# forbes110/taiwan-whisper

Measured on AMD Instinct MI355X. Metric: distillation utterances/sec (30 s clips), higher is better.
Workload: dtype bf16

## Files before the change

### include/tw_hip.h

```cpp
#ifndef TW_HIP_H
#define TW_HIP_H
#include <stdint.h>
#ifdef __cplusplus
extern "C" {
#endif

typedef void* tw_stream_t;

#define TW_GEMM_BIAS 1
#define TW_GEMM_ROUND 2
#define TW_GEMM_GELU 4
#define TW_GEMM_RES 8
#define TW_GEMM_ACCUM 16
#define TW_GEMM_AUX_OUT 32
#define TW_GEMM_DGELU 64
#define TW_GEMM_TILE128 256
#define TW_GEMM_TILE256 512
#define TW_GEMM_TILE256x128 1024
#define TW_GEMM_TILE256PP 2048
#define TW_GEMM_NOSPLIT 16384
#define TW_GEMM_TILE256x128_S2 262144
#define TW_GEMM_GROUP_M(g) ((g) << 24)


int tw_gemm_bf16(const void* A, int64_t lda, int a_trans, const void* B, int64_t ldb, int b_trans, void* C,
                 int64_t ldc, int c_dtype, int M, int N, int K, int batch, int64_t sA, int64_t sB, int64_t sC,
                 float alpha, const void* bias, const void* res, int64_t ldr, int64_t sR, int res_dtype, int res_mod,
                 void* aux, int64_t ldaux, int64_t sAux, int flags, tw_stream_t stream);

int tw_gemm_route(const void* A, int64_t lda, int a_trans, const void* B, int64_t ldb, int b_trans, void* C,
                  int64_t ldc, int c_dtype, int M, int N, int K, int batch, int64_t sA, int64_t sB, int64_t sC,
                  const void* bias, const void* res, int64_t ldr, int64_t sR, int res_dtype, int res_mod, void* aux,
                  int64_t ldaux, int64_t sAux, int flags, int is_f16, int cus, int have_ws, int* out);

int tw_gemv_bf16(const void* x, int64_t ldx, const float* ln_w, const float* ln_b, float eps, const void* W,
                 int64_t ldw, void* C, int64_t ldc, int c_dtype, int M, int N, int K, const void* bias,
                 const void* res, int64_t ldr, int res_dtype, void* aux, int64_t ldaux, int flags,
                 void* kv_cache, int64_t kv_sb, int64_t kv_ld, int kv_col0, const int* t_dev, tw_stream_t stream);

int tw_layernorm_fwd(const void* x, int x_dtype, const float* w, const float* b, void* y, int y_dtype,
                     float* mean_out, float* rstd_out, int rows, int D, float eps, tw_stream_t stream);
int tw_add_layernorm_fwd(const void* x, int x_dtype, const void* r, void* x_out, const float* w, const float* b,
                         void* y, float* mean_out, float* rstd_out, int rows, int D, float eps, tw_stream_t stream);
int tw_layernorm_bwd(const void* x, int x_dtype, const float* w, const float* mean, const float* rstd, const void* dy,
                     int dy_dtype, float* dx, int dx_accum, float* dw_out, float* db_out, int rows, int D,
                     float* workspace, int64_t workspace_floats, tw_stream_t stream);
int tw_layernorm_bwd_ex(const void* x, int x_dtype, const float* w, const float* mean, const float* rstd, const void* dy,
                        int dy_dtype, float* dx, int dx_accum, float* dw_out, float* db_out, int rows, int D,
                        float* workspace, int64_t workspace_floats, void* g16, int g_dtype, tw_stream_t stream);

int tw_attn_fwd(const void* Q, int64_t ldq, const void* K, int64_t ldk, const void* V, int64_t ldv, void* O,
                int64_t ldo, float* lse, int B, int H, int Tq, int Tk, int head_dim, int causal, float scale,
                tw_stream_t stream);
int tw_attn_bwd(const void* Q, int64_t ldq, const void* K, int64_t ldk, const void* V, int64_t ldv, const void* O,
                int64_t ldo, const void* dO, int64_t lddo, const float* lse, void* dQ, int64_t lddq, void* dK,
                int64_t lddk, void* dV, int64_t lddv, int B, int H, int Tq, int Tk, int head_dim, int causal,
                float scale, float* workspace , tw_stream_t stream);
int tw_attn_fwd_varlen(const void* Q, int64_t ldq, const void* K, int64_t ldk, const void* V, int64_t ldv, void* O,
                       int64_t ldo, float* lse, const int* offq, const int* offk, int B, int H, int Mq, int max_q, int Tk,
                       int head_dim, int causal, float scale, tw_stream_t stream);
int tw_attn_fwd_varlen_f16(const void* Q, int64_t ldq, const void* K, int64_t ldk, const void* V, int64_t ldv, void* O,
                           int64_t ldo, float* lse, const int* offq, const int* offk, int B, int H, int Mq, int max_q,
                           int Tk, int head_dim, int causal, float scale, tw_stream_t stream);
int tw_attn_bwd_varlen(const void* Q, int64_t ldq, const void* K, int64_t ldk, const void* V, int64_t ldv,
                       const void* O, int64_t ldo, const void* dO, int64_t lddo, const float* lse, void* dQ,
                       int64_t lddq, void* dK, int64_t lddk, void* dV, int64_t lddv, const int* offq, const int* offk,
// ... 111 lines not shown
int tw_gelu_bwd_f32(const float* g, const float* pre, float* out, int64_t n, tw_stream_t stream);

#define TW_GEMM_CLAMP16 128
int tw_gemm_f16(const void* A, int64_t lda, int a_trans, const void* B, int64_t ldb, int b_trans, void* C,
                int64_t ldc, int c_dtype, int M, int N, int K, int batch, int64_t sA, int64_t sB, int64_t sC,
                float alpha, const void* bias, const void* res, int64_t ldr, int64_t sR, int res_dtype, int res_mod,
                void* aux, int64_t ldaux, int64_t sAux, int flags, tw_stream_t stream);
int tw_gemv_f16(const void* x, int64_t ldx, const float* ln_w, const float* ln_b, float eps, const void* W,
                int64_t ldw, void* C, int64_t ldc, int c_dtype, int M, int N, int K, const void* bias,
                const void* res, int64_t ldr, int res_dtype, void* aux, int64_t ldaux, int flags,
                void* kv_cache, int64_t kv_sb, int64_t kv_ld, int kv_col0, const int* t_dev, tw_stream_t stream);
int tw_attn_fwd_f16(const void* Q, int64_t ldq, const void* K, int64_t ldk, const void* V, int64_t ldv, void* O,
                    int64_t ldo, float* lse, int B, int H, int Tq, int Tk, int head_dim, int causal, float scale,
                    tw_stream_t stream);
int tw_mel_to_conv_input_f16(const float* mel, void* xt, int B, int nmel, int T, tw_stream_t stream);
int tw_attn_bwd_f16(const void* Q, int64_t ldq, const void* K, int64_t ldk, const void* V, int64_t ldv, const void* O,
                    int64_t ldo, const void* dO, int64_t lddo, const float* lse, void* dQ, int64_t lddq, void* dK,
                    int64_t lddk, void* dV, int64_t lddv, int B, int H, int Tq, int Tk, int head_dim, int causal,
                    float scale, float* workspace, tw_stream_t stream);
int tw_gelu_bwd_f16(const void* g, int g_dtype, const void* pre, void* out, int64_t n, tw_stream_t stream);
int tw_cast_f32_f16(const float* src, void* dst, int64_t n, tw_stream_t stream);
int tw_add_layernorm_fwd_f16(const void* x, int x_dtype, const void* r, void* x_out, const float* w, const float* b,
                             void* y, float* mean_out, float* rstd_out, int rows, int D, float eps, tw_stream_t stream);
int tw_adamw_ex(float* p, const float* g, float* m, float* v, void* p16, int p16_dtype, int64_t n, float lr, float b1,
                float b2, float eps, float wd, int step, const float* norm, float max_norm, float inv_scale,
                tw_stream_t stream);

int tw_flac_info(const uint8_t* data, int64_t n, int64_t* info);
int tw_flac_decode(const uint8_t* data, int64_t n, int32_t* out, int64_t cap, int64_t* frames);

#ifdef __cplusplus
}
#endif
#endif
```

### taiwan-whisper_amd/csrc/layernorm.hip

```cpp
#include "common.h"

#include <algorithm>

namespace {

constexpr int WPB = 4;

template <int VEC, int MAXJ, bool ADD = false, bool RH = false>
__global__ __launch_bounds__(256) void ln_fwd_kernel(const void* __restrict__ x, int x_dtype,
                                                     const float* __restrict__ w, const float* __restrict__ b,
                                                     void* __restrict__ y, int y_dtype, float* __restrict__ mean_out,
                                                     float* __restrict__ rstd_out, int rows, int D, float eps,
                                                     const bf16* __restrict__ r = nullptr, float* x_out = nullptr) {
  const int lane = lane_id();
  const int row = blockIdx.x * WPB + (threadIdx.x >> 6);
  if (row >= rows) return;
  const int J = D / (64 * VEC);
  const int64_t base = (int64_t)row * D;
  float v[MAXJ][VEC];
  float s = 0.f;
#pragma unroll
  for (int j = 0; j < MAXJ; ++j) {
    if (j < J) {
      const int e = (j * 64 + lane) * VEC;
      if constexpr (ADD) {
        const f32x4 t = *(const f32x4*)((const float*)x + base + e);
        const bf16x4 u = *(const bf16x4*)(r + base + e);
        const f32x4 o = f32x4{t[0] + e2f<RH>(u[0]), t[1] + e2f<RH>(u[1]), t[2] + e2f<RH>(u[2]), t[3] + e2f<RH>(u[3])};
        *(f32x4*)(x_out + base + e) = o;
        v[j][0] = o[0]; v[j][1] = o[1]; v[j][2] = o[2]; v[j][3] = o[3];
      } else if (VEC == 4) {
        if (x_dtype == TW_F32) {
          f32x4 t = *(const f32x4*)((const float*)x + base + e);
          v[j][0] = t[0]; v[j][1] = t[1]; v[j][2] = t[2]; v[j][3] = t[3];
        } else if (x_dtype == TW_BF16) {
          bf16x4 t = *(const bf16x4*)((const bf16*)x + base + e);
          v[j][0] = bf2f(t[0]); v[j][1] = bf2f(t[1]); v[j][2] = bf2f(t[2]); v[j][3] = bf2f(t[3]);
        } else {
          f16x4 t = *(const f16x4*)((const f16*)x + base + e);
          v[j][0] = (float)t[0]; v[j][1] = (float)t[1]; v[j][2] = (float)t[2]; v[j][3] = (float)t[3];
        }
      } else {
        v[j][0] = ld_as_f32(x, x_dtype, base + e);
      }
#pragma unroll
      for (int q = 0; q < VEC; ++q) s += v[j][q];
    }
  }
  const float mean = wave_sum(s) / D;
  float ss = 0.f;
#pragma unroll
  for (int j = 0; j < MAXJ; ++j)
// ... 315 lines not shown
      default: hipLaunchKernelGGL((ln_fwd_bf16_kernel<5, true>), g2, block, 0, stream, xb, w, b, yb, mean_out, rstd_out,
                                  rows, D, eps, rb, xo); break;
    }
  }
  TW_CHECK_LAUNCH();
  return TW_OK;
}

extern "C" int tw_add_layernorm_fwd_f16(const void* x, int x_dtype, const void* r, void* x_out, const float* w,
                                        const float* b, void* y, float* mean_out, float* rstd_out, int rows, int D,
                                        float eps, hipStream_t stream) {
  if (rows <= 0) return TW_OK;
  if (D % 256 || D > 1280) return TW_EUNSUPPORTED;
  if (x_dtype != TW_F32) return TW_EUNSUPPORTED;
  if ((((uintptr_t)x | (uintptr_t)r | (uintptr_t)x_out | (uintptr_t)y | (uintptr_t)w | (uintptr_t)b) & 15) != 0)
    return TW_EINVAL;
  hipLaunchKernelGGL((ln_fwd_kernel<4, 5, true, true>), dim3((rows + WPB - 1) / WPB), dim3(64 * WPB), 0, stream, x,
                     (int)TW_F32, w, b, y, (int)TW_F16, mean_out, rstd_out, rows, D, eps, (const bf16*)r,
                     (float*)x_out);
  TW_CHECK_LAUNCH();
  return TW_OK;
}

extern "C" int tw_layernorm_bwd_ex(const void* x, int x_dtype, const float* w, const float* mean, const float* rstd,
                                   const void* dy, int dy_dtype, float* dx, int dx_accum, float* dw_out,
                                   float* db_out, int rows, int D, float* workspace, int64_t workspace_floats,
                                   void* g16, int g_dtype, hipStream_t stream) {
  if (rows <= 0) return TW_OK;
  if (g16 && g_dtype != TW_BF16 && g_dtype != TW_F16) return TW_EINVAL;
  if (D % 64 || D > 1280) return TW_EUNSUPPORTED;
  int nblk = (rows + WPB - 1) / WPB;
  if (nblk > 1024) nblk = 1024;
  if (workspace_floats < (int64_t)nblk * 2 * D) return TW_EINVAL;
  const bool v4 = D % 256 == 0 && (((uintptr_t)x | (uintptr_t)dy | (uintptr_t)dx | (uintptr_t)w | (uintptr_t)g16) & 15) == 0;
#define TW_LN_BWD(J)                                                                                          \
  hipLaunchKernelGGL((ln_bwd_kernel<4, J>), dim3(nblk), dim3(256), 0, stream, x, x_dtype, w, mean, rstd, dy, dy_dtype, \
                     dx, dx_accum, workspace, rows, D, g16, g_dtype)
  if (v4 && D > 1024) {
    static const int cap = [] {
      int dev = 0, cus = 0, per = 0;
      (void)hipGetDevice(&dev);
      (void)hipDeviceGetAttribute(&cus, hipDeviceAttributeMultiprocessorCount, dev);
      (void)hipOccupancyMaxActiveBlocksPerMultiprocessor(&per, (const void*)ln_bwd_kernel<4, 5>, 256, 0);
      return std::max(1, cus) * std::max(1, per);
    }();
    if (nblk > cap) nblk = cap;
// ... 24 lines not shown
```

### taiwan-whisper_amd/tw/_native.py

```python
from __future__ import annotations

import ctypes
import os

_HERE = os.path.dirname(os.path.abspath(__file__))
LIB_PATH = os.environ.get("TW_HIP_LIB", os.path.join(_HERE, "_lib", "libtw_hip.so"))

P, I64, I32, F32 = ctypes.c_void_p, ctypes.c_int64, ctypes.c_int, ctypes.c_float

SIGNATURES = {
    "tw_gemm_bf16": [P, I64, I32, P, I64, I32, P, I64, I32, I32, I32, I32, I32, I64, I64, I64, F32, P,
                     P, I64, I64, I32, I32, P, I64, I64, I32, P],
    "tw_gemm_route": [P, I64, I32, P, I64, I32, P, I64, I32, I32, I32, I32, I32, I64, I64, I64, P,
                      P, I64, I64, I32, I32, P, I64, I64, I32, I32, I32, I32, P],
    "tw_flac_info": [P, I64, P],
    "tw_flac_decode": [P, I64, P, I64, P],
    "tw_gemv_bf16": [P, I64, P, P, F32, P, I64, P, I64, I32, I32, I32, I32, P, P, I64, I32, P, I64, I32,
                     P, I64, I64, I32, P, P],
    "tw_layernorm_fwd": [P, I32, P, P, P, I32, P, P, I32, I32, F32, P],
    "tw_layernorm_bwd": [P, I32, P, P, P, P, I32, P, I32, P, P, I32, I32, P, I64, P],
    "tw_layernorm_bwd_ex": [P, I32, P, P, P, P, I32, P, I32, P, P, I32, I32, P, I64, P, I32, P],
    "tw_add_layernorm_fwd": [P, I32, P, P, P, P, P, P, P, I32, I32, F32, P],
    "tw_attn_fwd": [P, I64, P, I64, P, I64, P, I64, P, I32, I32, I32, I32, I32, I32, F32, P],
    "tw_attn_bwd": [P, I64, P, I64, P, I64, P, I64, P, I64, P, P, I64, P, I64, P, I64, I32, I32, I32, I32,
                    I32, I32, F32, P, P],
    "tw_attn_fwd_varlen": [P, I64, P, I64, P, I64, P, I64, P, P, P, I32, I32, I32, I32, I32, I32, I32, F32, P],
    "tw_attn_fwd_varlen_f16": [P, I64, P, I64, P, I64, P, I64, P, P, P, I32, I32, I32, I32, I32, I32, I32, F32, P],
    "tw_attn_bwd_varlen": [P, I64, P, I64, P, I64, P, I64, P, I64, P, P, I64, P, I64, P, I64, P, P, I32, I32, I32,
                           I32, I32, I32, I32, F32, P, P],
    "tw_attn_bwd_varlen_f16": [P, I64, P, I64, P, I64, P, I64, P, I64, P, P, I64, P, I64, P, I64, P, P, I32, I32,
                               I32, I32, I32, I32, I32, F32, P, P],
    "tw_pack_plan": [P, I32, I32, P, P, P],
    "tw_embed_fwd_rows": [P, P, P, I32, P, I32, P, I32, I32, I32, I32, I32, P],
    "tw_pos_grad_rows": [P, P, I32, I32, I32, P, P],
    "tw_kl_ce": [P, P, I64, I32, P, I64, I32, F32, F32, F32, P, F32, P, P, P, P],
    "tw_logmel": [P, I32, P, P, P, P, P, P, P],
    "tw_logmel_len": [P, I32, I64, P, P, P, P, P, P, P],
    "tw_logmel_mels": [P, I32, I64, I32, P, P, P, P, P, P, P],
    "tw_mel_to_conv_input": [P, P, I32, I32, I32, P],
    "tw_embed_fwd": [P, P, I32, P, I32, P, I32, I32, I32, I32, I32, P],
    "tw_embed_bwd": [P, P, P, I32, I32, I64, P],
    "tw_cast_f32_bf16": [P, P, I64, P],
    "tw_transpose_bf16": [P, I64, I32, I32, P, I64, P],
    "tw_colsum": [P, I32, I64, I32, I32, P, I32, I32, P, I64, P],
    "tw_l2norm": [P, I64, P, P, P],
# ... 12 lines not shown
    "tw_spec_accept": [P, I32, P, I32, I64, P, P, P, P, P, P, P, P, P, I32, I32, P, P, P, I32, P],
    "tw_embed_step_multi": [P, P, I32, P, I32, P, I32, I32, I32, P, I32, P],
    "tw_embed_step_off": [P, P, I32, P, I32, P, I32, I32, I32, P, P, P],
    "tw_greedy_select": [P, I64, I32, I32, I32, P, P, I32, I64, P, P, I64, I32, P, P, I32, P],
    "tw_greedy_select_ts": [P, I64, I32, I32, I32, P, P, I64, P, P, I64, I32, P, P, I32, I32, I32, I32, P, P],
    "tw_select_sample": [P, I64, I32, I32, I32, P, P, I32, I64, P, P, I64, I32, P, P, I32, P, P, P],
    "tw_select_sample_ts": [P, I64, I32, I32, I32, P, P, I64, P, P, I64, I32, P, P, I32, I32, I32, I32, P, P, P, P],
    "tw_token_logprob": [P, I64, I32, I32, I32, I32, P, P],
    "tw_embed_step": [P, P, I32, P, I32, P, I32, I32, I32, P, P],
    "tw_kv_append": [P, I64, P, I64, I64, I32, I32, I32, P, P],
    "tw_kv_head_major": [P, I64, P, I32, I32, I32, I32, P],
    "tw_step_advance": [P, I32, P],
    "tw_gemm_f16": [P, I64, I32, P, I64, I32, P, I64, I32, I32, I32, I32, I32, I64, I64, I64, F32, P,
                    P, I64, I64, I32, I32, P, I64, I64, I32, P],
    "tw_gemv_f16": [P, I64, P, P, F32, P, I64, P, I64, I32, I32, I32, I32, P, P, I64, I32, P, I64, I32,
                    P, I64, I64, I32, P, P],
    "tw_attn_fwd_f16": [P, I64, P, I64, P, I64, P, I64, P, I32, I32, I32, I32, I32, I32, F32, P],
    "tw_mel_to_conv_input_f16": [P, P, I32, I32, I32, P],
    "tw_attn_bwd_f16": [P, I64, P, I64, P, I64, P, I64, P, I64, P, P, I64, P, I64, P, I64, I32, I32, I32, I32,
                        I32, I32, F32, P, P],
    "tw_gelu_bwd_f16": [P, I32, P, P, I64, P],
    "tw_cast_f32_f16": [P, P, I64, P],
    "tw_add_layernorm_fwd_f16": [P, I32, P, P, P, P, P, P, P, I32, I32, F32, P],
    "tw_adamw_ex": [P, P, P, P, P, I32, I64, F32, F32, F32, F32, F32, I32, P, F32, F32, P],
    "tw_gemm_f32": [P, I64, I32, P, I64, I32, P, I64, I32, I32, I32, I32, I64, I64, I64, I32, I64, I64, I64, F32,
                    P, P, I64, I64, I32, P, I64, I64, I32, P],
    "tw_attn_fwd_f32": [P, I64, P, I64, P, I64, P, I64, P, I32, I32, I32, I32, I32, I32, F32, P, I64, P],
    "tw_attn_bwd_f32": [P, I64, P, I64, P, I64, P, I64, P, I64, P, P, I64, P, I64, P, I64, I32, I32, I32, I32, I32,
                        I32, F32, P, I64, P],
    "tw_mel_to_conv_input_f32": [P, P, I32, I32, I32, P],
    "tw_im2col3_f32": [P, I64, P, I32, I32, I32, I32, P],
    "tw_gelu_bwd_f32": [P, P, P, I64, P],
}

STATUS = {1: "invalid argument / shape", 2: "unsupported configuration", 3: "HIP launch error"}

_lib = None


def lib():
    global _lib
    if _lib is None:
        if not os.path.exists(LIB_PATH):
            raise RuntimeError(f"tw: HIP library not built: {LIB_PATH} (run `make -C taiwan-whisper_amd` "
                               "or __graft_entry__.build()); there is no CPU fallback")
        l = ctypes.CDLL(LIB_PATH)
# ... 14 lines not shown
```

### taiwan-whisper_amd/tw/distill.py

```python
from __future__ import annotations

import contextlib
import math
import os
from typing import Optional

import torch

from . import ops as F
from .modeling import Backward, PackedRows, WhisperForConditionalGeneration, is_pseudo


def constant_with_warmup(step: int, warmup: int) -> float:
    if warmup > 0 and step < warmup:
        return step / warmup
    return 1.0


def linear_schedule(step: int, warmup: int, total: int) -> float:
    if warmup > 0 and step < warmup:
        return step / warmup
    return max(0.0, (total - step) / max(1, total - warmup))


# ... 43 lines not shown
            if self.growth_tracker == self.growth_interval:
                self.scale *= self.growth_factor
                self.growth_tracker = 0

    def state_dict(self):
        return {"scale": self.scale, "growth_factor": self.growth_factor, "backoff_factor": self.backoff_factor,
                "growth_interval": self.growth_interval, "_growth_tracker": self.growth_tracker}

    def load_state_dict(self, sd):
        self.scale = float(sd["scale"])
        self.growth_factor, self.backoff_factor = float(sd["growth_factor"]), float(sd["backoff_factor"])
        self.growth_interval = int(sd["growth_interval"])
        self.growth_tracker = int(sd["_growth_tracker"])


class DistillationTrainer:
    def __init__(self, student: WhisperForConditionalGeneration, teacher: WhisperForConditionalGeneration, *,
                 temperature: float = 2.0, kl_weight: float = 1.0, learning_rate: float = 1e-4,
                 adam_beta1: float = 0.9, adam_beta2: float = 0.999, adam_epsilon: float = 1e-8,
                 weight_decay: float = 0.0, max_grad_norm: float = 1.0, warmup_steps: int = 0,
                 lr_scheduler_type: str = "constant_with_warmup", max_steps: int = 0,
                 gradient_accumulation_steps: int = 1, freeze_encoder: bool = True, freeze_decoder: bool = False,
                 freeze_embed_positions: bool = True, process_group=None, dp_bucket_mb: int = 64,
                 overlap_update: Optional[bool] = None, force_exchange: bool = False):
        if student.compute != teacher.compute:
            raise ValueError(f"student computes in {student.compute}, teacher in {teacher.compute}: the reference "
                             "runs both under one mixed_precision setting")
        self.s, self.t = student, teacher
        self.temperature, self.kl_weight = temperature, kl_weight
        self.lr, self.b1, self.b2, self.eps = learning_rate, adam_beta1, adam_beta2, adam_epsilon
        self.wd, self.max_grad_norm = weight_decay, max_grad_norm
        self.warmup, self.sched, self.max_steps = warmup_steps, lr_scheduler_type, max_steps
        self.accum = gradient_accumulation_steps
        self.pg = process_group
        self.world = torch.distributed.get_world_size(process_group) if process_group is not None else 1
        self.force_exchange = bool(force_exchange) and process_group is not None
        self.dp = self.world > 1 or self.force_exchange
        self.bucket = dp_bucket_mb * (1 << 20) // 4
        self.fold_world = self.world & (self.world - 1) == 0
        self.overlap_update = (self.dp and freeze_encoder) if overlap_update is None else bool(overlap_update)
        if self.overlap_update and not freeze_encoder:
            raise ValueError("overlap_update needs a frozen encoder: the next forward must read no trainable weight")
        self.scaler = GradScaler() if student.compute == "fp16" else None
        if self.scaler is not None:
            if student.dtype != torch.float32:
                raise ValueError("fp16 distillation trains an fp32-master student under fp16 autocast")
            if overlap_update:
                raise ValueError("overlap_update: the fp16 loss scaler decides each update on the host")
            self.overlap_update = False
        self.pack_rows = student.compute != "fp32" and os.environ.get("TW_PACK_ROWS", "1") != "0"
        self._pin = {}
# ... 24 lines not shown
        return weight_decay_runs(self.s, self.wd, self.freeze_encoder, self.freeze_decoder)

    def num_trainable_parameters(self):
        return self.s.num_parameters(only_trainable=True)

    def lr_at(self, step):
        if self.sched == "linear":
            return self.lr * linear_schedule(step, self.warmup, self.max_steps)
        if self.sched == "constant":
            return self.lr
        return self.lr * constant_with_warmup(step, self.warmup)

    def _conv_input(self, batch):
        ci = batch.get("conv_input")
        if ci is not None and ci.dtype == self.s.act_dtype:
            return ci
        return self.s.conv_input(batch["input_features"])

    def _teacher_logits(self, conv_in, ids, labels, enc16, Tk, pk=None):
        t = self.t
        if self.share:
            t_ids = torch.empty_like(labels)
            F.shift_tokens_right(labels, t_ids, t.config.pad_token_id, t.config.decoder_start_token_id)
            ht = t.decode(t_ids if pk is None else pk.pack(t_ids), enc16, Tk, pk=pk)
        else:
            enc_t = t.encode(conv_in)
            ht = t.decode(ids if pk is None else pk.pack(ids), enc_t, Tk, pk=pk)
        return t.lm_head(ht)

    def _plan_rows(self, batch_labels, labels):
        B, T = labels.shape
        off = torch.empty(B + 1, dtype=torch.int32, device=labels.device)
        src = torch.empty(B * T, dtype=torch.int64, device=labels.device)
        F.pack_plan(labels, off, src)
        def descriptor(lens):
            pk = PackedRows(lens, off, src, T)
            return pk if pk.M > 0 else None

        if not batch_labels.is_cuda:
            pos = torch.arange(1, T + 1, dtype=torch.int64)
            lens = ((batch_labels >= 0) * pos).amax(1).tolist()
            return lambda: descriptor(lens)
        host = self._pin.get(B)
        if host is None:
            host = self._pin[B] = torch.empty(B + 1, dtype=torch.int32).pin_memory()
        host.copy_(off, non_blocking=True)
        ev = torch.cuda.Event()
        ev.record()

        def done():
            ev.synchronize()
            o = host.tolist()
            return descriptor([o[b + 1] - o[b] for b in range(B)])
        return done

    def train_step(self, batch, temperature: Optional[float] = None, end_of_dataloader: bool = False):
        T = self.temperature if temperature is None else temperature
        s = self.s
        conv_in = self._conv_input(batch)
        ids = batch["decoder_input_ids"].to(s.device).contiguous()
        labels = batch["labels"].to(s.device).contiguous()
        B, Td = ids.shape
        plan = self._plan_rows(batch["labels"], labels) if self.pack_rows else None
        enc_tape = [] if self.train_encoder else None
        enc16 = s.encode(conv_in, tape=enc_tape)
        self.flush()
        pk = plan() if plan is not None else None
        if self.micro == 0:
            s.grad.zero_()
        self._pending, self._reduced = [], []
        sync = self.micro + 1 == self.accum or end_of_dataloader
        self.bw.on_ready = self._grad_ready if (self.dp and sync) else None
        Tk = enc16.shape[0] // B
        tape = []
        with self._row_capacity(pk, B * Td):
            hs = s.decode(ids if pk is None else pk.pack(ids), enc16, Tk, tape=tape, pk=pk)
            ls = s.lm_head(hs)
            with torch.no_grad():
                lt = self._teacher_logits(conv_in, ids, labels, enc16, Tk, pk)
            lab = labels.reshape(-1) if pk is None else pk.pack(labels)
            F.count_valid(lab, self.nvalid)
            dlogits = ls
            gs = (self.scaler.scale if self.scaler is not None else 1.0) / (self.accum * (self.world if self.fold_world
                                                                                             else 1))
            out3, _ = F.kl_ce(ls, lt, lab, s.config.vocab_size, self.nvalid, T=T, ce_w=0.8, kl_w=self.kl_weight,
                              grad_scale=gs, dlogits=dlogits)
            del lt
            d_enc = torch.zeros(B * Tk, s.config.d_model, dtype=torch.float32, device=s.device) \
                if self.train_encoder else None
            self.bw.decoder(tape, dlogits, hs, enc16, d_enc)
            del tape, dlogits, ls
        if self.train_encoder:
            self.bw.encoder(enc_tape, d_enc)
        self.micro += 1
        if sync:
            self.optimizer_step()
            self.micro = 0
        return {"loss": out3[0], "ce_loss": out3[1], "kl_loss": out3[2]}

    def _row_capacity(self, pk, cap):
        ctx = contextlib.ExitStack()
        if pk is not None:
            ctx.enter_context(self.s.row_capacity(cap))
            ctx.enter_context(self.t.row_capacity(cap))
        return ctx

    def eval_step(self, batch):
        self.flush()
        s = self.s
        conv_in = self._conv_input(batch)
        ids = batch["decoder_input_ids"].to(s.device).contiguous()
        labels = batch["labels"].to(s.device).contiguous()
        B, Td = ids.shape
        plan = self._plan_rows(batch["labels"], labels) if self.pack_rows else None
        enc16 = s.encode(conv_in)
        pk = plan() if plan is not None else None
        Tk = enc16.shape[0] // B
        with self._row_capacity(pk, B * Td):
            ls = s.lm_head(s.decode(ids if pk is None else pk.pack(ids), enc16, Tk, pk=pk))
            lt = self._teacher_logits(conv_in, ids, labels, enc16, Tk, pk)
            lab = labels.reshape(-1) if pk is None else pk.pack(labels)
            nv = torch.zeros(1, dtype=torch.int32, device=s.device)
            F.count_valid(lab, nv)
            out3, _ = F.kl_ce(ls, lt, lab, s.config.vocab_size, nv, T=1.0, ce_w=0.8, kl_w=self.kl_weight)
        return {"loss": out3[0], "ce_loss": out3[1], "kl_loss": out3[2]}

    def _launch(self, lo, hi, tail=False):
        g = self.s.grad
        for a in range(lo, hi, self.bucket):
            sl = g[a: min(hi, a + self.bucket)]
            if not self.fold_world:
                sl.mul_(1.0 / self.world)
            self._pending.append((torch.distributed.all_reduce(sl, group=self.pg, async_op=True), tail))
            if getattr(self, "exchange_log", None) is not None:
                self.exchange_log.append((sl.numel() * sl.element_size(), tail))
        self._reduced.append((lo, hi))

    def _grad_ready(self, prefix):
        r = self.s.grad_range(prefix)
        if r is not None:
            self._launch(*r)

# ... 176 lines not shown
```

### taiwan-whisper_amd/tw/modeling.py

```python
from __future__ import annotations

import json
import math
import os
from dataclasses import dataclass
from typing import Optional

import numpy as np
import torch

from . import ops
from .config import GenerationConfig, WhisperConfig

_DEFER_RES = os.environ.get("TW_DEFER_RES", "1")
_LN_G16 = os.environ.get("TW_LN_G16", "1") != "0"

F = ops


def padded_vocab(V: int) -> int:
    return (V + 63) // 64 * 64



# ... 402 lines not shown
        N, K = w.shape
        F.gemm(x, w, out, M, N, K, lda=x.stride(0), ldb=K, ldc=out.stride(0), bias=b, res=res,
               ldr=res.stride(0) if res is not None else 0, aux=aux, ldaux=aux.stride(0) if aux is not None else 0,
               flags=flags)
        return out

    def _ln(self, x, name, out_dtype=None, save=None):
        y = self._rows(x.shape[0], x.shape[1], out_dtype or self.act_dtype)
        mean = rstd = None
        if save is not None:
            mean = torch.empty(x.shape[0], dtype=torch.float32, device=self.device)
            rstd = torch.empty_like(mean)
            save[name] = (x, mean, rstd, y)
        F.layernorm_fwd(x, self.ln_param(name + ".weight"), self.ln_param(name + ".bias"), y, mean, rstd)
        return y

    def defer_residual(self, kind):
        if _DEFER_RES == "0" or self.act_dtype == torch.float32 or self.config.d_model % 256 or self.config.d_model > 1280:
            return False
        if self.act_dtype == torch.float16:
            return self.stream_dtype == torch.float32
        return self.stream_dtype == torch.float32 or (kind == "attn" and _DEFER_RES != "2")

    def _ln_in(self, x, pend, name, save):
        if pend is None:
            return x, self._ln(x, name, save=save)
        xn = x if save is None else self._rows(x.shape[0], x.shape[1], x.dtype)
        y = self._rows(x.shape[0], x.shape[1], self.act_dtype)
        mean = rstd = None
        if save is not None:
            mean = torch.empty(x.shape[0], dtype=torch.float32, device=self.device)
            rstd = torch.empty_like(mean)
            save[name] = (xn, mean, rstd, y)
        F.add_layernorm_fwd(x, pend, xn, self.ln_param(name + ".weight"), self.ln_param(name + ".bias"), y, mean, rstd)
        return xn, y

    def _res_out(self, h, w, b, x, tape, kind, clamp=False):
        M, N = h.shape[0], w.shape[0]
        if self.defer_residual(kind):
            r = self._rows(M, N, self.act_dtype)
            self._lin(h, w, b, r)
            return x, r
        out = self._rows(M, N, self.stream_dtype) if tape is not None else x
        flags = F.GEMM_ROUND | (F.GEMM_CLAMP16 if clamp and self.stream_dtype == torch.float16 else 0)
        self._lin(h, w, b, out, res=x, flags=flags)
        return out, None

    def _attn_fwd(self, x, p, q, ldq, k, v, ldkv, B, T, Tk, causal, tape, pk):
        d = self.config.d_model
        H = d // 64
        M = B * T if pk is None else pk.M
        o = self._rows(M, d, self.act_dtype)
        lse = torch.empty(H * M, dtype=torch.float32, device=self.device) if tape is not None else None
        if pk is None:
            F.attn_fwd(q, ldq, k, ldkv, v, ldkv, o, d, lse, B, H, T, T if Tk is None else Tk, causal, 0.125)
        else:
            offk, Tk = (pk.off, pk.max_len) if Tk is None else (None, Tk)
            F.attn_fwd_varlen(q, ldq, k, ldkv, v, ldkv, o, d, lse, pk.off, offk, pk.B, H, M, pk.max_len, Tk, causal, 0.125)
        out = self._res_out(o, self._w16(p + ".out_proj.weight"), self._w16(p + ".out_proj.bias"), x, tape, "attn")
        return out, o, lse

    def _attn_block(self, x, p, B, T, causal, tape=None, pend=None, pk=None):
        d = self.config.d_model
        sv = {} if tape is not None else None
        x, y = self._ln_in(x, pend, p + "_layer_norm", sv)
        M = B * T if pk is None else pk.M
        qkv = self._rows(M, 3 * d, self.act_dtype)
        wqkv = self.wspan(p + ".q_proj.weight", p + ".v_proj.weight", (3 * d, d))
        bqkv = self.wspan(p + ".q_proj.bias", p + ".v_proj.bias", (3 * d,))
        self._lin(y, wqkv, bqkv, qkv)
        out, o, lse = self._attn_fwd(x, p, qkv, 3 * d, qkv[:, d:], qkv[:, 2 * d:], 3 * d, B, T, None, causal, tape, pk)
        if tape is not None:
            tape.append(("attn", p, dict(sv=sv, y=y, qkv=qkv, o=o, lse=lse, B=B, T=T, causal=causal, pk=pk)))
        return out

    def _cross_block(self, x, enc16, p, B, T, Tk, tape=None, kv=None, pend=None, pk=None):
        d = self.config.d_model
        sv = {} if tape is not None else None
        x, y = self._ln_in(x, pend, p + "_layer_norm", sv)
        M = B * T if pk is None else pk.M
        q = self._rows(M, d, self.act_dtype)
        self._lin(y, self._w16(p + ".q_proj.weight"), self._w16(p + ".q_proj.bias"), q)
        if kv is None:
            kv = torch.empty(B * Tk, 2 * d, dtype=self.act_dtype, device=self.device)
            wkv = self.wspan(p + ".k_proj.weight", p + ".v_proj.weight", (2 * d, d))
            bkv = self.wspan(p + ".k_proj.zero_bias", p + ".v_proj.bias", (2 * d,))
            self._lin(enc16, wkv, bkv, kv)
        out, o, lse = self._attn_fwd(x, p, q, d, kv, kv[:, d:], 2 * d, B, T, Tk, False, tape, pk)
        if tape is not None:
            tape.append(("cross", p, dict(sv=sv, y=y, q=q, kv=kv, o=o, lse=lse, B=B, T=T, Tk=Tk, pk=pk)))
        return out

    def _mlp_block(self, x, p, tape=None, pend=None, clamp=False):
        M = x.shape[0]
        sv = {} if tape is not None else None
        x, y = self._ln_in(x, pend, p + ".final_layer_norm", sv)
        f = self.store.segs[p + ".fc1.weight"][0]
        h = self._rows(M, f, self.act_dtype)
        pre = self._rows(M, f, self.act_dtype) if tape is not None else None
        self._lin(y, self._w16(p + ".fc1.weight"), self._w16(p + ".fc1.bias"), h, aux=pre,
                  flags=F.GEMM_ROUND | F.GEMM_GELU | (F.GEMM_AUX_OUT if tape is not None else 0))
        out = self._res_out(h, self._w16(p + ".fc2.weight"), self._w16(p + ".fc2.bias"), x, tape, "mlp", clamp=clamp)
        if tape is not None:
            tape.append(("mlp", p, dict(sv=sv, y=y, h=h, pre=pre)))
        return out

    def conv_input(self, input_features: torch.Tensor) -> torch.Tensor:
        B, nm, T = input_features.shape
        if T != 2 * self.config.max_source_positions:
            raise ValueError(f"Whisper expects the mel input features to be of length "
                             f"{2 * self.config.max_source_positions}, but found {T}.")
        xt = torch.empty(B, T + 2, nm, dtype=self.act_dtype, device=self.device)
        F.mel_to_conv_input(input_features.to(self.device, torch.float32).contiguous(), xt)
        return xt

    def encode(self, conv_in: torch.Tensor, tape=None) -> torch.Tensor:
        cfg, d = self.config, self.config.d_model
        B, T2 = conv_in.shape[0], conv_in.shape[1] - 2
        T = T2 // 2
        nm = cfg.num_mel_bins
        if conv_in.dtype != self.act_dtype:
            raise ValueError(f"conv input is {conv_in.dtype}, this model computes in {self.act_dtype}")
        H1 = torch.empty(B, T2 + 2, d, dtype=self.act_dtype, device=self.device)
        H1[:, 0].zero_()
        H1[:, T2 + 1].zero_()
        pre1 = pre2 = None
        if tape is not None:
            pre1 = torch.empty(B, T2, d, dtype=self.act_dtype, device=self.device)
            pre2 = torch.empty(B, T, d, dtype=self.act_dtype, device=self.device)
        gf = F.GEMM_ROUND | F.GEMM_GELU | (F.GEMM_AUX_OUT if tape is not None else 0)
        F.gemm(conv_in, self._w16("model.encoder.conv1.weight"), H1[:, 1:], T2, d, 3 * nm, lda=nm, ldb=3 * nm,
               ldc=d, batch=B, sA=(T2 + 2) * nm, sC=(T2 + 2) * d, bias=self._w16("model.encoder.conv1.bias"),
               aux=pre1, ldaux=d, sAux=T2 * d, flags=gf)
        x = torch.empty(B * T, d, dtype=self.stream_dtype, device=self.device)
        pos = self.store.v32("model.encoder.embed_positions.weight") if self.store.p32 is not None \
            else self.store.v16("model.encoder.embed_positions.weight")
        F.gemm(H1, self._w16("model.encoder.conv2.weight"), x, T, d, 3 * d, lda=2 * d, ldb=3 * d, ldc=d, batch=B,
               sA=(T2 + 2) * d, sC=T * d, bias=self._w16("model.encoder.conv2.bias"), res=pos, ldr=d, res_mod=T,
               aux=pre2, ldaux=d, sAux=T * d, flags=gf)
        if tape is not None:
            tape.append(("conv", "model.encoder", dict(conv_in=conv_in, H1=H1, pre1=pre1, pre2=pre2, B=B, T=T)))
        pend = None
        for i in range(cfg.encoder_layers):
            p = f"model.encoder.layers.{i}"
            x, pend = self._attn_block(x, p + ".self_attn", B, T, False, tape, pend)
            x, pend = self._mlp_block(x, p, tape, pend, clamp=True)
        sv = {} if tape is not None else None
        _, enc = self._ln_in(x, pend, "model.encoder.layer_norm", sv)
        if tape is not None:
            tape.append(("ln_final", "model.encoder.layer_norm", dict(sv=sv)))
        return enc

    def embed(self, ids: torch.Tensor, pk=None) -> torch.Tensor:
        d = self.config.d_model
        if self.store.p32 is not None:
            tok, pos = self.store.v32("model.decoder.embed_tokens.weight"), self.store.v32(
                "model.decoder.embed_positions.weight")
        else:
            tok, pos = self.store.v16("model.decoder.embed_tokens.weight"), self.store.v16(
                "model.decoder.embed_positions.weight")
        if pk is not None:
            return F.embed_fwd_rows(ids, pk.src, tok, pos, self._rows(pk.M, d, self.stream_dtype), pk.T)
        B, T = ids.shape
        x = torch.empty(B * T, d, dtype=self.stream_dtype, device=self.device)
        F.embed_fwd(ids.reshape(-1).contiguous(), tok, pos, x, T)
        return x

    def decode(self, ids: torch.Tensor, enc16: torch.Tensor, Tk: int, tape=None, pk=None) -> torch.Tensor:
        cfg = self.config
        if pk is not None:
            if self.compute == "fp32":
                raise ValueError("packed rows: the fp32-compute path keeps padded rows")
            B, T = pk.B, pk.T
            if ids.dim() != 1 or ids.numel() != pk.M or enc16.shape[0] != B * Tk:
                raise ValueError("packed rows: ids must be the packed [M] ids and enc16 hold B*Tk rows")
        else:
            B, T = ids.shape
        if T > cfg.max_target_positions:
            raise ValueError("decoder input longer than max_target_positions")
        ids = ids.contiguous()
        x = self.embed(ids, pk)
        if tape is not None:
            tape.append(("embed", "model.decoder", dict(ids=ids.reshape(-1), B=B, T=T, pk=pk)))
        pend = None
        for i in range(cfg.decoder_layers):
            p = f"model.decoder.layers.{i}"
            x, pend = self._attn_block(x, p + ".self_attn", B, T, True, tape, pend, pk=pk)
            x, pend = self._cross_block(x, enc16, p + ".encoder_attn", B, T, Tk, tape, pend=pend, pk=pk)
            x, pend = self._mlp_block(x, p, tape, pend)
        sv = {} if tape is not None else None
        _, h = self._ln_in(x, pend, "model.decoder.layer_norm", sv)
        if tape is not None:
            tape.append(("ln_final", "model.decoder.layer_norm", dict(sv=sv)))
        return h

    def lm_head(self, h16: torch.Tensor, out=None) -> torch.Tensor:
        M = h16.shape[0]
        if out is None:
            out = self._rows(M, self.Vp, self.act_dtype)
        E = self._w16("model.decoder.embed_tokens.weight")
        F.gemm(h16, E, out, M, self.Vp, self.config.d_model, lda=h16.stride(0), ldb=self.config.d_model,
               ldc=self.Vp, flags=F.GEMM_ROUND, algo_N=self.config.vocab_size)
        return out

    def __call__(self, input_features=None, decoder_input_ids=None, labels=None, encoder_outputs=None,
                 conv_input=None, **kw) -> Seq2SeqOutput:
        cfg = self.config
        if encoder_outputs is not None:
            enc = encoder_outputs.last_hidden_state if hasattr(encoder_outputs, "last_hidden_state") \
                else encoder_outputs[0]
            B = enc.shape[0]
            enc16 = enc.reshape(-1, cfg.d_model).to(self.device, self.act_dtype).contiguous()
            Tk = enc.shape[1]
        else:
# ... 289 lines not shown
```

### taiwan-whisper_amd/tw/ops.py

```python
from __future__ import annotations

import collections
import ctypes

import torch

from ._native import call
from .profiling import KernelTimer

F32, BF16, F16 = 0, 1, 2
GEMM_BIAS, GEMM_ROUND, GEMM_GELU, GEMM_RES, GEMM_ACCUM, GEMM_AUX_OUT, GEMM_DGELU = 1, 2, 4, 8, 16, 32, 64
GEMM_CLAMP16 = 128
HALF = (torch.bfloat16, torch.float16)
GEMM_TILE128, GEMM_TILE256, GEMM_TILE256x128, GEMM_TILE256PP = 256, 512, 1024, 2048
GEMM_NOSPLIT = 16384
GEMM_TILE256x128_S2 = 262144


def GEMM_GROUP_M(g: int) -> int:
    assert 0 < g < 16
    return g << 24


GEMM_ROUTES = ("skinny", "skinny_splitk", "splitk_dw", "rounds_sk_tail", "rounds_dp_tail", "persistent",
# ... 135 lines not shown
        _need(mean, rows, "ln mean"); _need(rstd, rows, "ln rstd")
    call("tw_layernorm_fwd", x.data_ptr(), _dt(x), w.data_ptr(), b.data_ptr(), y.data_ptr(), _dt(y),
         _ptr(mean), _ptr(rstd), rows, D, float(eps), _stream())
    return y


def add_layernorm_fwd(x, r, x_out, w, b, y, mean=None, rstd=None, eps=1e-5):
    D = x.shape[-1]
    rows = x.numel() // D
    h = r.dtype
    assert h in HALF and y.dtype == h and x_out.dtype == x.dtype
    assert x.dtype in ((torch.float32, torch.bfloat16) if h == torch.bfloat16 else (torch.float32,))
    for t in (x, r, x_out, y):
        assert t.is_contiguous() and t.numel() == x.numel() and t.is_cuda
    assert w.dtype == torch.float32 and b.dtype == torch.float32 and w.numel() == D and b.numel() == D
    if mean is not None:
        _need(mean, rows, "ln mean"); _need(rstd, rows, "ln rstd")
    call("tw_add_layernorm_fwd_f16" if h == torch.float16 else "tw_add_layernorm_fwd", x.data_ptr(), _dt(x),
         r.data_ptr(), x_out.data_ptr(), w.data_ptr(), b.data_ptr(),
         y.data_ptr(), _ptr(mean), _ptr(rstd), rows, D, float(eps), _stream())
    return y


def layernorm_bwd(x, w, mean, rstd, dy, dx, dw, db, dx_accum=True, workspace=None, g16=None):
    D = x.shape[-1]
    rows = x.numel() // D
    assert dx.dtype == torch.float32 and dx.numel() == x.numel() and dy.numel() == x.numel()
    nblk = min(1024, (rows + 3) // 4)
    if workspace is None or workspace.numel() < nblk * 2 * D:
        workspace = torch.empty(nblk * 2 * D, dtype=torch.float32, device=x.device)
    if g16 is None:
        call("tw_layernorm_bwd", x.data_ptr(), _dt(x), w.data_ptr(), mean.data_ptr(), rstd.data_ptr(), dy.data_ptr(),
             _dt(dy), dx.data_ptr(), int(dx_accum), _ptr(dw), _ptr(db), rows, D, workspace.data_ptr(),
             workspace.numel(), _stream())
        return dx
    assert g16.dtype in HALF and g16.is_contiguous() and g16.numel() == dx.numel() and dx.is_contiguous()
    call("tw_layernorm_bwd_ex", x.data_ptr(), _dt(x), w.data_ptr(), mean.data_ptr(), rstd.data_ptr(), dy.data_ptr(),
         _dt(dy), dx.data_ptr(), int(dx_accum), _ptr(dw), _ptr(db), rows, D, workspace.data_ptr(), workspace.numel(),
         g16.data_ptr(), _dt(g16), _stream())
    return dx


def _attn_sym(name, q, q_side, k_side, lse, H, B, Tq, Tk, offq=None, offk=None, Mq=None):
    if Mq is None:
        rows_q, rows_k, n_lse = B * Tq, B * Tk, B * H * Tq
    else:
# ... 556 lines not shown
```

Baseline: 269.0.

## Chain deferred residuals through fused add-LayerNorm to skip fp32 stream writes

```diff
diff --git a/include/tw_hip.h b/include/tw_hip.h
--- a/include/tw_hip.h
+++ b/include/tw_hip.h
@@ -42,6 +42,9 @@
                      float* mean_out, float* rstd_out, int rows, int D, float eps, tw_stream_t stream);
 int tw_add_layernorm_fwd(const void* x, int x_dtype, const void* r, void* x_out, const float* w, const float* b,
                          void* y, float* mean_out, float* rstd_out, int rows, int D, float eps, tw_stream_t stream);
+int tw_add_layernorm_fwd_ex(const void* x, int x_dtype, const void* r, const void* r2, void* x_out, const float* w,
+                            const float* b, void* y, float* mean_out, float* rstd_out, int rows, int D, float eps,
+                            tw_stream_t stream);
 int tw_layernorm_bwd(const void* x, int x_dtype, const float* w, const float* mean, const float* rstd, const void* dy,
                      int dy_dtype, float* dx, int dx_accum, float* dw_out, float* db_out, int rows, int D,
                      float* workspace, int64_t workspace_floats, tw_stream_t stream);
@@ -199,6 +202,9 @@
 int tw_cast_f32_f16(const float* src, void* dst, int64_t n, tw_stream_t stream);
 int tw_add_layernorm_fwd_f16(const void* x, int x_dtype, const void* r, void* x_out, const float* w, const float* b,
                              void* y, float* mean_out, float* rstd_out, int rows, int D, float eps, tw_stream_t stream);
+int tw_add_layernorm_fwd_ex_f16(const void* x, int x_dtype, const void* r, const void* r2, void* x_out, const float* w,
+                                const float* b, void* y, float* mean_out, float* rstd_out, int rows, int D, float eps,
+                                tw_stream_t stream);
 int tw_adamw_ex(float* p, const float* g, float* m, float* v, void* p16, int p16_dtype, int64_t n, float lr, float b1,
                 float b2, float eps, float wd, int step, const float* norm, float max_norm, float inv_scale,
                 tw_stream_t stream);
diff --git a/taiwan-whisper_amd/csrc/layernorm.hip b/taiwan-whisper_amd/csrc/layernorm.hip
--- a/taiwan-whisper_amd/csrc/layernorm.hip
+++ b/taiwan-whisper_amd/csrc/layernorm.hip
@@ -6,16 +6,17 @@
 
 constexpr int WPB = 4;
 
-template <int VEC, int MAXJ, bool ADD = false, bool RH = false>
+template <int VEC, int MAXJ, bool ADD = false, bool RH = false, bool WR = true, bool R2 = false, bool EX = false>
 __global__ __launch_bounds__(256) void ln_fwd_kernel(const void* __restrict__ x, int x_dtype,
                                                      const float* __restrict__ w, const float* __restrict__ b,
                                                      void* __restrict__ y, int y_dtype, float* __restrict__ mean_out,
                                                      float* __restrict__ rstd_out, int rows, int D, float eps,
-                                                     const bf16* __restrict__ r = nullptr, float* x_out = nullptr) {
+                                                     const bf16* __restrict__ r = nullptr, float* x_out = nullptr,
+                                                     const bf16* __restrict__ r2 = nullptr) {
   const int lane = lane_id();
   const int row = blockIdx.x * WPB + (threadIdx.x >> 6);
   if (row >= rows) return;
-  const int J = D / (64 * VEC);
+  const int J = EX ? MAXJ : D / (64 * VEC);
   const int64_t base = (int64_t)row * D;
   float v[MAXJ][VEC];
   float s = 0.f;
@@ -26,8 +27,12 @@
       if constexpr (ADD) {
         const f32x4 t = *(const f32x4*)((const float*)x + base + e);
         const bf16x4 u = *(const bf16x4*)(r + base + e);
-        const f32x4 o = f32x4{t[0] + e2f<RH>(u[0]), t[1] + e2f<RH>(u[1]), t[2] + e2f<RH>(u[2]), t[3] + e2f<RH>(u[3])};
-        *(f32x4*)(x_out + base + e) = o;
+        f32x4 o = f32x4{t[0] + e2f<RH>(u[0]), t[1] + e2f<RH>(u[1]), t[2] + e2f<RH>(u[2]), t[3] + e2f<RH>(u[3])};
+        if constexpr (R2) {
+          const bf16x4 u2 = *(const bf16x4*)(r2 + base + e);
+          o = f32x4{o[0] + e2f<RH>(u2[0]), o[1] + e2f<RH>(u2[1]), o[2] + e2f<RH>(u2[2]), o[3] + e2f<RH>(u2[3])};
+        }
+        if constexpr (WR) *(f32x4*)(x_out + base + e) = o;
         v[j][0] = o[0]; v[j][1] = o[1]; v[j][2] = o[2]; v[j][3] = o[3];
       } else if (VEC == 4) {
         if (x_dtype == TW_F32) {
@@ -389,6 +394,53 @@
   return TW_OK;
 }
 
+namespace {
+
+template <bool RH>
+int add_ln_chain(const void* x, int x_dtype, const void* r, const void* r2, void* x_out, const float* w, const float* b,
+                 void* y, float* mean_out, float* rstd_out, int rows, int D, float eps, hipStream_t stream) {
+  if (rows <= 0) return TW_OK;
+  if (D % 256 || D > 1280 || x_dtype != TW_F32) return TW_EUNSUPPORTED;
+  if (!x || !r || !y || (r2 && !x_out)) return TW_EINVAL;
+  if ((((uintptr_t)x | (uintptr_t)r | (uintptr_t)r2 | (uintptr_t)x_out | (uintptr_t)y | (uintptr_t)w | (uintptr_t)b) &
+       15) != 0)
+    return TW_EINVAL;
+  const dim3 grid((rows + WPB - 1) / WPB), block(64 * WPB);
+  const int yd = RH ? (int)TW_F16 : (int)TW_BF16;
+#define TW_LN_CHAIN(J, WR, R2)                                                                                        \
+  hipLaunchKernelGGL((ln_fwd_kernel<4, J, true, RH, WR, R2, true>), grid, block, 0, stream, x, (int)TW_F32, w, b, y, \
+                     yd, mean_out, rstd_out, rows, D, eps, (const bf16*)r, (float*)x_out, (const bf16*)r2)
+#define TW_LN_CHAIN_J(J)                  \
+  if (r2) TW_LN_CHAIN(J, true, true);     \
+  else if (x_out) TW_LN_CHAIN(J, true, false); \
+  else TW_LN_CHAIN(J, false, false)
+  switch (D / 256) {
+    case 1: TW_LN_CHAIN_J(1); break;
+    case 2: TW_LN_CHAIN_J(2); break;
+    case 3: TW_LN_CHAIN_J(3); break;
+    case 4: TW_LN_CHAIN_J(4); break;
+    default: TW_LN_CHAIN_J(5); break;
+  }
+#undef TW_LN_CHAIN_J
+#undef TW_LN_CHAIN
+  TW_CHECK_LAUNCH();
+  return TW_OK;
+}
+
+}
+
+extern "C" int tw_add_layernorm_fwd_ex(const void* x, int x_dtype, const void* r, const void* r2, void* x_out,
+                                       const float* w, const float* b, void* y, float* mean_out, float* rstd_out,
+                                       int rows, int D, float eps, hipStream_t stream) {
+  return add_ln_chain<false>(x, x_dtype, r, r2, x_out, w, b, y, mean_out, rstd_out, rows, D, eps, stream);
+}
+
+extern "C" int tw_add_layernorm_fwd_ex_f16(const void* x, int x_dtype, const void* r, const void* r2, void* x_out,
+                                           const float* w, const float* b, void* y, float* mean_out, float* rstd_out,
+                                           int rows, int D, float eps, hipStream_t stream) {
+  return add_ln_chain<true>(x, x_dtype, r, r2, x_out, w, b, y, mean_out, rstd_out, rows, D, eps, stream);
+}
+
 extern "C" int tw_layernorm_bwd_ex(const void* x, int x_dtype, const float* w, const float* mean, const float* rstd,
                                    const void* dy, int dy_dtype, float* dx, int dx_accum, float* dw_out,
                                    float* db_out, int rows, int D, float* workspace, int64_t workspace_floats,
diff --git a/taiwan-whisper_amd/tw/_native.py b/taiwan-whisper_amd/tw/_native.py
--- a/taiwan-whisper_amd/tw/_native.py
+++ b/taiwan-whisper_amd/tw/_native.py
@@ -21,6 +21,7 @@
     "tw_layernorm_bwd": [P, I32, P, P, P, P, I32, P, I32, P, P, I32, I32, P, I64, P],
     "tw_layernorm_bwd_ex": [P, I32, P, P, P, P, I32, P, I32, P, P, I32, I32, P, I64, P, I32, P],
     "tw_add_layernorm_fwd": [P, I32, P, P, P, P, P, P, P, I32, I32, F32, P],
+    "tw_add_layernorm_fwd_ex": [P, I32, P, P, P, P, P, P, P, P, I32, I32, F32, P],
     "tw_attn_fwd": [P, I64, P, I64, P, I64, P, I64, P, I32, I32, I32, I32, I32, I32, F32, P],
     "tw_attn_bwd": [P, I64, P, I64, P, I64, P, I64, P, I64, P, P, I64, P, I64, P, I64, I32, I32, I32, I32,
                     I32, I32, F32, P, P],
@@ -79,6 +80,7 @@
     "tw_gelu_bwd_f16": [P, I32, P, P, I64, P],
     "tw_cast_f32_f16": [P, P, I64, P],
     "tw_add_layernorm_fwd_f16": [P, I32, P, P, P, P, P, P, P, I32, I32, F32, P],
+    "tw_add_layernorm_fwd_ex_f16": [P, I32, P, P, P, P, P, P, P, P, I32, I32, F32, P],
     "tw_adamw_ex": [P, P, P, P, P, I32, I64, F32, F32, F32, F32, F32, I32, P, F32, F32, P],
     "tw_gemm_f32": [P, I64, I32, P, I64, I32, P, I64, I32, I32, I32, I32, I64, I64, I64, I32, I64, I64, I64, F32,
                     P, P, I64, I64, I32, P, I64, I64, I32, P],
diff --git a/taiwan-whisper_amd/tw/distill.py b/taiwan-whisper_amd/tw/distill.py
--- a/taiwan-whisper_amd/tw/distill.py
+++ b/taiwan-whisper_amd/tw/distill.py
@@ -89,11 +89,12 @@
                  lr_scheduler_type: str = "constant_with_warmup", max_steps: int = 0,
                  gradient_accumulation_steps: int = 1, freeze_encoder: bool = True, freeze_decoder: bool = False,
                  freeze_embed_positions: bool = True, process_group=None, dp_bucket_mb: int = 64,
-                 overlap_update: Optional[bool] = None, force_exchange: bool = False):
+                 overlap_update: Optional[bool] = None, force_exchange: bool = False, ln_chain: bool = True):
         if student.compute != teacher.compute:
             raise ValueError(f"student computes in {student.compute}, teacher in {teacher.compute}: the reference "
                              "runs both under one mixed_precision setting")
         self.s, self.t = student, teacher
+        self.ln_chain = bool(ln_chain)
         self.temperature, self.kl_weight = temperature, kl_weight
         self.lr, self.b1, self.b2, self.eps = learning_rate, adam_beta1, adam_beta2, adam_epsilon
         self.wd, self.max_grad_norm = weight_decay, max_grad_norm
@@ -164,10 +165,10 @@
         if self.share:
             t_ids = torch.empty_like(labels)
             F.shift_tokens_right(labels, t_ids, t.config.pad_token_id, t.config.decoder_start_token_id)
-            ht = t.decode(t_ids if pk is None else pk.pack(t_ids), enc16, Tk, pk=pk)
+            ht = t.decode(t_ids if pk is None else pk.pack(t_ids), enc16, Tk, pk=pk, chain=self.ln_chain)
         else:
-            enc_t = t.encode(conv_in)
-            ht = t.decode(ids if pk is None else pk.pack(ids), enc_t, Tk, pk=pk)
+            enc_t = t.encode(conv_in, chain=self.ln_chain)
+            ht = t.decode(ids if pk is None else pk.pack(ids), enc_t, Tk, pk=pk, chain=self.ln_chain)
         return t.lm_head(ht)
 
     def _plan_rows(self, batch_labels, labels):
@@ -205,7 +206,7 @@
         B, Td = ids.shape
         plan = self._plan_rows(batch["labels"], labels) if self.pack_rows else None
         enc_tape = [] if self.train_encoder else None
-        enc16 = s.encode(conv_in, tape=enc_tape)
+        enc16 = s.encode(conv_in, tape=enc_tape, chain=self.ln_chain)
         self.flush()
         pk = plan() if plan is not None else None
         if self.micro == 0:
@@ -216,7 +217,7 @@
         Tk = enc16.shape[0] // B
         tape = []
         with self._row_capacity(pk, B * Td):
-            hs = s.decode(ids if pk is None else pk.pack(ids), enc16, Tk, tape=tape, pk=pk)
+            hs = s.decode(ids if pk is None else pk.pack(ids), enc16, Tk, tape=tape, pk=pk, chain=self.ln_chain)
             ls = s.lm_head(hs)
             with torch.no_grad():
                 lt = self._teacher_logits(conv_in, ids, labels, enc16, Tk, pk)
@@ -255,11 +256,11 @@
         labels = batch["labels"].to(s.device).contiguous()
         B, Td = ids.shape
         plan = self._plan_rows(batch["labels"], labels) if self.pack_rows else None
-        enc16 = s.encode(conv_in)
+        enc16 = s.encode(conv_in, chain=self.ln_chain)
         pk = plan() if plan is not None else None
         Tk = enc16.shape[0] // B
         with self._row_capacity(pk, B * Td):
-            ls = s.lm_head(s.decode(ids if pk is None else pk.pack(ids), enc16, Tk, pk=pk))
+            ls = s.lm_head(s.decode(ids if pk is None else pk.pack(ids), enc16, Tk, pk=pk, chain=self.ln_chain))
             lt = self._teacher_logits(conv_in, ids, labels, enc16, Tk, pk)
             lab = labels.reshape(-1) if pk is None else pk.pack(labels)
             nv = torch.zeros(1, dtype=torch.int32, device=s.device)
diff --git a/taiwan-whisper_amd/tw/modeling.py b/taiwan-whisper_amd/tw/modeling.py
--- a/taiwan-whisper_amd/tw/modeling.py
+++ b/taiwan-whisper_amd/tw/modeling.py
@@ -448,9 +448,16 @@
             return self.stream_dtype == torch.float32
         return self.stream_dtype == torch.float32 or (kind == "attn" and _DEFER_RES != "2")
 
-    def _ln_in(self, x, pend, name, save):
+    def _ln_in(self, x, pend, name, save, chain=False):
         if pend is None:
-            return x, self._ln(x, name, save=save)
+            return x, self._ln(x, name, save=save), None
+        if isinstance(pend, tuple) or (chain and save is None and x.dtype == torch.float32):
+            assert save is None and x.dtype == torch.float32
+            r1, r2 = pend if isinstance(pend, tuple) else (pend, None)
+            y = self._rows(x.shape[0], x.shape[1], self.act_dtype)
+            F.add_layernorm_chain_fwd(x, r1, r2, x if r2 is not None else None, self.ln_param(name + ".weight"),
+                                      self.ln_param(name + ".bias"), y)
+            return x, y, (r1 if r2 is None else None)
         xn = x if save is None else self._rows(x.shape[0], x.shape[1], x.dtype)
         y = self._rows(x.shape[0], x.shape[1], self.act_dtype)
         mean = rstd = None
@@ -459,20 +466,21 @@
             rstd = torch.empty_like(mean)
             save[name] = (xn, mean, rstd, y)
         F.add_layernorm_fwd(x, pend, xn, self.ln_param(name + ".weight"), self.ln_param(name + ".bias"), y, mean, rstd)
-        return xn, y
-
-    def _res_out(self, h, w, b, x, tape, kind, clamp=False):
+        return xn, y, None
+
+    def _res_out(self, h, w, b, x, tape, kind, clamp=False, keep=None):
         M, N = h.shape[0], w.shape[0]
         if self.defer_residual(kind):
             r = self._rows(M, N, self.act_dtype)
             self._lin(h, w, b, r)
-            return x, r
+            return x, (r if keep is None else (keep, r))
+        assert keep is None
         out = self._rows(M, N, self.stream_dtype) if tape is not None else x
         flags = F.GEMM_ROUND | (F.GEMM_CLAMP16 if clamp and self.stream_dtype == torch.float16 else 0)
         self._lin(h, w, b, out, res=x, flags=flags)
         return out, None
 
-    def _attn_fwd(self, x, p, q, ldq, k, v, ldkv, B, T, Tk, causal, tape, pk):
+    def _attn_fwd(self, x, p, q, ldq, k, v, ldkv, B, T, Tk, causal, tape, pk, keep=None):
         d = self.config.d_model
         H = d // 64
         M = B * T if pk is None else pk.M
@@ -483,27 +491,29 @@
         else:
             offk, Tk = (pk.off, pk.max_len) if Tk is None else (None, Tk)
             F.attn_fwd_varlen(q, ldq, k, ldkv, v, ldkv, o, d, lse, pk.off, offk, pk.B, H, M, pk.max_len, Tk, causal, 0.125)
-        out = self._res_out(o, self._w16(p + ".out_proj.weight"), self._w16(p + ".out_proj.bias"), x, tape, "attn")
+        out = self._res_out(o, self._w16(p + ".out_proj.weight"), self._w16(p + ".out_proj.bias"), x, tape, "attn",
+                            keep=keep)
         return out, o, lse
 
-    def _attn_block(self, x, p, B, T, causal, tape=None, pend=None, pk=None):
+    def _attn_block(self, x, p, B, T, causal, tape=None, pend=None, pk=None, chain=False):
         d = self.config.d_model
         sv = {} if tape is not None else None
-        x, y = self._ln_in(x, pend, p + "_layer_norm", sv)
+        x, y, keep = self._ln_in(x, pend, p + "_layer_norm", sv, chain)
         M = B * T if pk is None else pk.M
         qkv = self._rows(M, 3 * d, self.act_dtype)
         wqkv = self.wspan(p + ".q_proj.weight", p + ".v_proj.weight", (3 * d, d))
         bqkv = self.wspan(p + ".q_proj.bias", p + ".v_proj.bias", (3 * d,))
         self._lin(y, wqkv, bqkv, qkv)
-        out, o, lse = self._attn_fwd(x, p, qkv, 3 * d, qkv[:, d:], qkv[:, 2 * d:], 3 * d, B, T, None, causal, tape, pk)
+        out, o, lse = self._attn_fwd(x, p, qkv, 3 * d, qkv[:, d:], qkv[:, 2 * d:], 3 * d, B, T, None, causal, tape, pk,
+                                     keep)
         if tape is not None:
             tape.append(("attn", p, dict(sv=sv, y=y, qkv=qkv, o=o, lse=lse, B=B, T=T, causal=causal, pk=pk)))
         return out
 
-    def _cross_block(self, x, enc16, p, B, T, Tk, tape=None, kv=None, pend=None, pk=None):
+    def _cross_block(self, x, enc16, p, B, T, Tk, tape=None, kv=None, pend=None, pk=None, chain=False):
         d = self.config.d_model
         sv = {} if tape is not None else None
-        x, y = self._ln_in(x, pend, p + "_layer_norm", sv)
+        x, y, keep = self._ln_in(x, pend, p + "_layer_norm", sv, chain)
         M = B * T if pk is None else pk.M
         q = self._rows(M, d, self.act_dtype)
         self._lin(y, self._w16(p + ".q_proj.weight"), self._w16(p + ".q_proj.bias"), q)
@@ -512,21 +522,22 @@
             wkv = self.wspan(p + ".k_proj.weight", p + ".v_proj.weight", (2 * d, d))
             bkv = self.wspan(p + ".k_proj.zero_bias", p + ".v_proj.bias", (2 * d,))
             self._lin(enc16, wkv, bkv, kv)
-        out, o, lse = self._attn_fwd(x, p, q, d, kv, kv[:, d:], 2 * d, B, T, Tk, False, tape, pk)
+        out, o, lse = self._attn_fwd(x, p, q, d, kv, kv[:, d:], 2 * d, B, T, Tk, False, tape, pk, keep)
         if tape is not None:
             tape.append(("cross", p, dict(sv=sv, y=y, q=q, kv=kv, o=o, lse=lse, B=B, T=T, Tk=Tk, pk=pk)))
         return out
 
-    def _mlp_block(self, x, p, tape=None, pend=None, clamp=False):
+    def _mlp_block(self, x, p, tape=None, pend=None, clamp=False, chain=False):
         M = x.shape[0]
         sv = {} if tape is not None else None
-        x, y = self._ln_in(x, pend, p + ".final_layer_norm", sv)
+        x, y, keep = self._ln_in(x, pend, p + ".final_layer_norm", sv, chain)
         f = self.store.segs[p + ".fc1.weight"][0]
         h = self._rows(M, f, self.act_dtype)
         pre = self._rows(M, f, self.act_dtype) if tape is not None else None
         self._lin(y, self._w16(p + ".fc1.weight"), self._w16(p + ".fc1.bias"), h, aux=pre,
                   flags=F.GEMM_ROUND | F.GEMM_GELU | (F.GEMM_AUX_OUT if tape is not None else 0))
-        out = self._res_out(h, self._w16(p + ".fc2.weight"), self._w16(p + ".fc2.bias"), x, tape, "mlp", clamp=clamp)
+        out = self._res_out(h, self._w16(p + ".fc2.weight"), self._w16(p + ".fc2.bias"), x, tape, "mlp", clamp=clamp,
+                            keep=keep)
         if tape is not None:
             tape.append(("mlp", p, dict(sv=sv, y=y, h=h, pre=pre)))
         return out
@@ -540,7 +551,7 @@
         F.mel_to_conv_input(input_features.to(self.device, torch.float32).contiguous(), xt)
         return xt
 
-    def encode(self, conv_in: torch.Tensor, tape=None) -> torch.Tensor:
+    def encode(self, conv_in: torch.Tensor, tape=None, chain=True) -> torch.Tensor:
         cfg, d = self.config, self.config.d_model
         B, T2 = conv_in.shape[0], conv_in.shape[1] - 2
         T = T2 // 2
@@ -569,10 +580,10 @@
         pend = None
         for i in range(cfg.encoder_layers):
             p = f"model.encoder.layers.{i}"
-            x, pend = self._attn_block(x, p + ".self_attn", B, T, False, tape, pend)
-            x, pend = self._mlp_block(x, p, tape, pend, clamp=True)
+            x, pend = self._attn_block(x, p + ".self_attn", B, T, False, tape, pend, chain=chain)
+            x, pend = self._mlp_block(x, p, tape, pend, clamp=True, chain=chain)
         sv = {} if tape is not None else None
-        _, enc = self._ln_in(x, pend, "model.encoder.layer_norm", sv)
+        _, enc, _ = self._ln_in(x, pend, "model.encoder.layer_norm", sv, chain)
         if tape is not None:
             tape.append(("ln_final", "model.encoder.layer_norm", dict(sv=sv)))
         return enc
@@ -592,7 +603,7 @@
         F.embed_fwd(ids.reshape(-1).contiguous(), tok, pos, x, T)
         return x
 
-    def decode(self, ids: torch.Tensor, enc16: torch.Tensor, Tk: int, tape=None, pk=None) -> torch.Tensor:
+    def decode(self, ids: torch.Tensor, enc16: torch.Tensor, Tk: int, tape=None, pk=None, chain=True) -> torch.Tensor:
         cfg = self.config
         if pk is not None:
             if self.compute == "fp32":
@@ -611,11 +622,11 @@
         pend = None
         for i in range(cfg.decoder_layers):
             p = f"model.decoder.layers.{i}"
-            x, pend = self._attn_block(x, p + ".self_attn", B, T, True, tape, pend, pk=pk)
-            x, pend = self._cross_block(x, enc16, p + ".encoder_attn", B, T, Tk, tape, pend=pend, pk=pk)
-            x, pend = self._mlp_block(x, p, tape, pend)
+            x, pend = self._attn_block(x, p + ".self_attn", B, T, True, tape, pend, pk=pk, chain=chain)
+            x, pend = self._cross_block(x, enc16, p + ".encoder_attn", B, T, Tk, tape, pend=pend, pk=pk, chain=chain)
+            x, pend = self._mlp_block(x, p, tape, pend, chain=chain)
         sv = {} if tape is not None else None
-        _, h = self._ln_in(x, pend, "model.decoder.layer_norm", sv)
+        _, h, _ = self._ln_in(x, pend, "model.decoder.layer_norm", sv, chain)
         if tape is not None:
             tape.append(("ln_final", "model.decoder.layer_norm", dict(sv=sv)))
         return h
diff --git a/taiwan-whisper_amd/tw/ops.py b/taiwan-whisper_amd/tw/ops.py
--- a/taiwan-whisper_amd/tw/ops.py
+++ b/taiwan-whisper_amd/tw/ops.py
@@ -181,6 +181,24 @@
     return y
 
 
+def add_layernorm_chain_fwd(x, r, r2, x_out, w, b, y, mean=None, rstd=None, eps=1e-5):
+    D = x.shape[-1]
+    rows = x.numel() // D
+    h = r.dtype
+    assert h in HALF and y.dtype == h and x.dtype == torch.float32
+    assert r2 is None or (r2.dtype == h and x_out is not None)
+    assert x_out is None or x_out.dtype == torch.float32
+    for t in (x, r, r2, x_out, y):
+        assert t is None or (t.is_contiguous() and t.numel() == x.numel() and t.is_cuda)
+    assert w.dtype == torch.float32 and b.dtype == torch.float32 and w.numel() == D and b.numel() == D
+    if mean is not None:
+        _need(mean, rows, "ln mean"); _need(rstd, rows, "ln rstd")
+    call("tw_add_layernorm_fwd_ex_f16" if h == torch.float16 else "tw_add_layernorm_fwd_ex", x.data_ptr(), _dt(x),
+         r.data_ptr(), _ptr(r2), _ptr(x_out), w.data_ptr(), b.data_ptr(), y.data_ptr(), _ptr(mean), _ptr(rstd), rows, D,
+         float(eps), _stream())
+    return y
+
+
 def layernorm_bwd(x, w, mean, rstd, dy, dx, dw, db, dx_accum=True, workspace=None, g16=None):
     D = x.shape[-1]
     rows = x.numel() // D
```

Result: no change. 270.4, median of 6 (+0.5%).
